# LiyaoTang/contrastBoundary

Hardware: AMD Instinct MI355X
Metric: points/sec through KNN+group+KPConv+CBL block, S3DIS N=40960 K=16 (higher is better)
Workload: dtype f32

## Files before the change

contrastboundary_amd/build.py:

```python
import concurrent.futures
import os
import shutil
import subprocess
import sys

PKG = os.path.dirname(os.path.abspath(__file__))
CSRC = os.path.join(PKG, "csrc")
LIBDIR = os.path.join(PKG, "lib")
OBJDIR = os.path.join(LIBDIR, "obj")
SO = os.path.join(LIBDIR, "libcbl_amd.so")
INCLUDE = os.path.join(os.path.dirname(PKG), "include")

HIPCC = shutil.which("hipcc") or "/opt/rocm/bin/hipcc"
FLAGS = ["--offload-arch=gfx950", "-O3", "-std=c++17", "-fPIC", "-ffp-contract=off", "-munsafe-fp-atomics",
         "-fvisibility=hidden", "-Wall", "-Wno-unused-function", "-I" + INCLUDE, "-I" + CSRC]


def sources():
    return sorted(os.path.join(CSRC, f) for f in os.listdir(CSRC) if f.endswith(".hip"))


def headers():
    hs = [os.path.join(CSRC, f) for f in os.listdir(CSRC) if f.endswith(".h")]
    hs += [os.path.join(INCLUDE, f) for f in os.listdir(INCLUDE) if f.endswith(".h")]
    return hs


EXTRA_FLAGS = {"local_aggregation.hip": ["-mllvm", "-amdgpu-mfma-vgpr-form"]}

def _compile(src, obj, verbose):
    tmp = obj + ".tmp.%d" % os.getpid()
    cmd = [HIPCC] + FLAGS + EXTRA_FLAGS.get(os.path.basename(src), []) + ["-c", src, "-o", tmp]
    if verbose:
        print(" ".join(cmd), flush=True)
    r = subprocess.run(cmd, capture_output=True, text=True)
    if r.returncode != 0:
        raise RuntimeError("hipcc failed for %s:\n%s\n%s" % (src, r.stdout, r.stderr))
    if verbose and r.stderr.strip():
        print(r.stderr)
    os.replace(tmp, obj)


def is_stale():
    if not os.path.exists(SO):
        return True
    t = os.path.getmtime(SO)
    return any(os.path.getmtime(p) > t for p in sources() + headers())


def build(force=False, verbose=False):
    import fcntl
    os.makedirs(OBJDIR, exist_ok=True)
    with open(os.path.join(LIBDIR, ".build.lock"), "w") as lock:
        fcntl.flock(lock, fcntl.LOCK_EX)
        try:
            if not force and not is_stale():
                return SO
            return _build_locked(force, verbose)
        finally:
            fcntl.flock(lock, fcntl.LOCK_UN)


def _build_locked(force, verbose):
    hdr_time = max([os.path.getmtime(h) for h in headers()] + [os.path.getmtime(__file__)])
    jobs, objs = [], []
    for src in sources():
        obj = os.path.join(OBJDIR, os.path.basename(src)[:-4] + ".o")
        objs.append(obj)
        if force or not os.path.exists(obj) or os.path.getmtime(obj) < max(os.path.getmtime(src), hdr_time):
            jobs.append((src, obj))
    if jobs:
        with concurrent.futures.ThreadPoolExecutor(max_workers=min(8, len(jobs))) as ex:
            for f in [ex.submit(_compile, s, o, verbose) for s, o in jobs]:
                f.result()
    if jobs or not os.path.exists(SO):
        tmp = SO + ".tmp.%d" % os.getpid()
        cmd = [HIPCC, "--offload-arch=gfx950", "-shared", "-fPIC", "-o", tmp] + objs
        if verbose:
            print(" ".join(cmd), flush=True)
        r = subprocess.run(cmd, capture_output=True, text=True)
        if r.returncode != 0:
            raise RuntimeError("link failed:\n%s\n%s" % (r.stdout, r.stderr))
        os.replace(tmp, SO)
    else:
        os.utime(SO)
    return SO


if __name__ == "__main__":
    print(build(force="--force" in sys.argv, verbose="--verbose" in sys.argv))
```

contrastboundary_amd/hotpath.py:

```python
import os
import sys

import torch

from . import heads, local_aggregation, pointops

KP = 15
CBL_NSAMPLE = 36
CBL_DIM = 32


class Scene:

    def __init__(self, xyz, feat, labels, offset):
        self.xyz, self.feat, self.labels, self.offset = xyz, feat, labels, offset
        self.n, self.c = feat.shape

    @staticmethod
    def synthetic_numpy(n, c, seed=0, b=1):
        import numpy as np
        from . import synthetic as S
        xyz, labels = S.s_room(n, seed, scale=1.0 if n <= 100000 else float(np.sqrt(n / 40000.0)))
        rng = np.random.default_rng(seed + 1000)
        feat = rng.normal(size=(n, c)).astype(np.float32)
        off = S.offsets(n, b, seed)
        kpts = (rng.normal(size=(KP, 3)) * 0.06).astype(np.float32); kpts[0] = 0
        kw = (rng.normal(size=(KP, c)) / np.sqrt(KP)).astype(np.float32)
        latent = rng.normal(size=(n, CBL_DIM)).astype(np.float32)
        return dict(xyz=xyz, feat=feat, labels=labels, offset=off, kernel_points=kpts, kernel_weights=kw, latent=latent)

    @staticmethod
    def upstream_numpy(n, c, k, seed=0):
        import numpy as np
        rng = np.random.default_rng(seed + 2000)
        return dict(grad_grouped=rng.normal(size=(n, k, 3 + c)).astype(np.float32), grad_kpconv=rng.normal(size=(n, c)).astype(np.float32))

    @staticmethod
    def synthetic(n, c, seed=0, b=1, device="cuda"):
        a = Scene.synthetic_numpy(n, c, seed, b)
        t = lambda v: torch.from_numpy(v).to(device)
        sc = Scene(t(a["xyz"]), t(a["feat"]), t(a["labels"]), t(a["offset"]))
        sc.kernel_points, sc.kernel_weights, sc.latent = t(a["kernel_points"]), t(a["kernel_weights"]), t(a["latent"])
        sc.seed = seed
        return sc

    def upstream(self, k):
        cache = self.__dict__.setdefault("_upstream", {})
        if k not in cache:
            a = Scene.upstream_numpy(self.n, self.c, k, getattr(self, "seed", 0))
            cache[k] = {name: torch.from_numpy(v).to(self.xyz.device) for name, v in a.items()}
        return cache[k]


SIDE_STAGES = ("cbl_knnquery_k%d" % CBL_NSAMPLE,)


def stages(scene, k=16, backward=False, pair_tables=False):
    n, c = scene.n, scene.c
    st = []
    leaf = (lambda t: t.detach().requires_grad_(True)) if backward else (lambda t: t)
    if backward:
        scene.upstream(k)

    def knn(s):
        s["idx"], s["dist2"] = pointops.knnquery_raw(k, scene.xyz, scene.xyz, scene.offset, scene.offset)
    st.append(("knnquery_k%d" % k, knn, 12 * n + 12 * n + 8 * n * k, 8.0 * n * n))

    def group(s):
        s["feat_leaf"], s["kw_leaf"] = leaf(scene.feat), leaf(scene.kernel_weights)
        s["grouped"] = pointops.queryandgroup(k, scene.xyz, scene.xyz, s["feat_leaf"], s["idx"], scene.offset, scene.offset, use_xyz=True)
    st.append(("queryandgroup", group, 4 * n * k + 12 * n + 12 * n + 4 * n * c + 4 * n * k * (3 + c), 3.0 * n * k))

    extent = 0.12

    def kpconv(s):
        s["kpconv"] = local_aggregation.kpconv(scene.xyz, scene.xyz, s["idx"], s["feat_leaf"], scene.kernel_points, s["kw_leaf"], extent)
    st.append(("kpconv_fwd", kpconv, 12 * n + 12 * n + 4 * n * c + 4 * n * k + 4 * n * c, 2.0 * n * k * KP * c + 2.0 * n * KP * c))

    d = CBL_DIM

    def cbl_knn(s):
        s["cbl_idx"], _ = pointops.knnquery_raw(CBL_NSAMPLE, scene.xyz, scene.xyz, scene.offset, scene.offset, algo="set")
    st.append(("cbl_knnquery_k%d" % CBL_NSAMPLE, cbl_knn, 24 * n + 8 * n * CBL_NSAMPLE, 8.0 * n * n))

    def cbl_transpose(s):
        s["cbl_transposed"] = pointops.neighbor_transpose(s["cbl_idx"], n, companion=s.get("idx") if (pair_tables and backward) else None)
    st.append(("cbl_neighbor_transpose", cbl_transpose, 8 * n * CBL_NSAMPLE + 4 * (n + 1), 0.0))

    def cbl_fwd(s):
        s["cbl_latent"] = scene.latent.detach().requires_grad_(True)
        s["cbl_loss"] = heads.point_contrast(s["cbl_latent"], scene.labels, s["cbl_idx"], 1.0, 0.1)
    st.append(("cbl_mining_loss_fwd", cbl_fwd, 4 * n * CBL_NSAMPLE + 4 * n * d + 4 * n + 8 * n + 4 * n * CBL_NSAMPLE + 4 * n * d,
               1.0 * n * (CBL_NSAMPLE - 1) * (8 * d + 50)))

    def cbl_bwd(s):
        s["cbl_grad"], = torch.autograd.grad(s["cbl_loss"], s["cbl_latent"])
    st.append(("cbl_mining_loss_bwd", cbl_bwd, 4 * (n + 1) + 8 * n * CBL_NSAMPLE + 12 * n * d, 3.0 * n * (CBL_NSAMPLE - 1) * d))
    if not backward:
        return st

    def transpose(s):
        s["transposed"] = pointops.neighbor_transpose(s["idx"], n)
    st.append(("neighbor_transpose_k%d" % k, transpose, 8 * n * k + 4 * (n + 1), 0.0))

    def group_bwd(s):
        s["grad_feat_group"], = torch.autograd.grad(s["grouped"], s["feat_leaf"], scene.upstream(k)["grad_grouped"])
    st.append(("queryandgroup_bwd", group_bwd, 4 * n * k + 4 * n * k * c + 4 * n * c, 1.0 * n * k * c))

    def kpconv_bwd(s):
        s["grad_feat_kpconv"], s["grad_kernel_weights"] = torch.autograd.grad(s["kpconv"], (s["feat_leaf"], s["kw_leaf"]), scene.upstream(k)["grad_kpconv"])
    st.append(("kpconv_bwd", kpconv_bwd, 12 * n + 12 * n + 4 * n * c + 4 * n * k + 4 * n * c + 4 * n * c + 4 * KP * c,
               2.0 * (2.0 * n * k * KP * c + 2.0 * n * KP * c)))
    return st


def pt_layer(scene, seed=0):
    from . import blocks
    cache = scene.__dict__.setdefault("_pt_layer", {})
    if seed not in cache:
        torch.manual_seed(1234 + seed)
        cache[seed] = blocks.PointTransformerLayer(scene.c, scene.c, 8, 16).to(scene.xyz.device).train()
    return cache[seed]


def stages_pt(scene, k=16, backward=False, pair_tables=False):
    n, c = scene.n, scene.c
    layer = pt_layer(scene)
    layer.nsample = k
    params = [p for p in layer.parameters()]
    st = []
    if backward:
        scene.upstream(k)

    def knn(s):
        s["idx"], s["dist2"] = pointops.knnquery_raw(k, scene.xyz, scene.xyz, scene.offset, scene.offset)
    st.append(("knnquery_k%d" % k, knn, 12 * n + 12 * n + 8 * n * k, 8.0 * n * n))

    def layer_fwd(s):
        s["feat_leaf"] = scene.feat.detach().requires_grad_(True) if backward else scene.feat
        s["pt_out"] = layer([scene.xyz, s["feat_leaf"], scene.offset], idx=s["idx"])
    st.append(("pt_layer_fwd", layer_fwd, 12 * n + 12 * n * c + 4 * n * k + 4 * n * c,
               2.0 * n * k * (9 + 3 * c + c * c / 8.0 + c * c / 64.0) + 6.0 * n * c * c))

    d = CBL_DIM

    def cbl_knn(s):
        s["cbl_idx"], _ = pointops.knnquery_raw(CBL_NSAMPLE, scene.xyz, scene.xyz, scene.offset, scene.offset, algo="set")
    st.append(("cbl_knnquery_k%d" % CBL_NSAMPLE, cbl_knn, 24 * n + 8 * n * CBL_NSAMPLE, 8.0 * n * n))

    def cbl_transpose(s):
        s["cbl_transposed"] = pointops.neighbor_transpose(s["cbl_idx"], n, companion=s.get("idx") if (pair_tables and backward) else None)
    st.append(("cbl_neighbor_transpose", cbl_transpose, 8 * n * CBL_NSAMPLE + 4 * (n + 1), 0.0))

    def cbl_fwd(s):
        s["cbl_latent"] = scene.latent.detach().requires_grad_(True)
        s["cbl_loss"] = heads.point_contrast(s["cbl_latent"], scene.labels, s["cbl_idx"], 1.0, 0.1)
    st.append(("cbl_mining_loss_fwd", cbl_fwd, 4 * n * CBL_NSAMPLE + 4 * n * d + 4 * n + 8 * n + 4 * n * CBL_NSAMPLE + 4 * n * d,
               1.0 * n * (CBL_NSAMPLE - 1) * (8 * d + 50)))

# ... 315 lines not shown
```

contrastboundary_amd/local_aggregation.py:

```python
import collections
import ctypes

import torch
from torch.autograd import Function

from . import _lib

_i = ctypes.c_int
_f = ctypes.c_float


def _chk(t, dtype, name):
    if not (isinstance(t, torch.Tensor) and t.is_cuda and t.dtype == dtype and t.is_contiguous()):
        raise TypeError(f"{name}: expected a contiguous CUDA tensor of {dtype}")
    return t


class _KPConv(Function):
    @staticmethod
    def forward(ctx, query_points, support_points, neighbors_indices, features, kernel_points, kernel_weights, extent, influence, closest):
        n, K = neighbors_indices.shape
        n0, C = features.shape
        KP = kernel_points.shape[0]
        out = torch.empty((n, C), dtype=torch.float32, device=features.device)
        from . import pointops
        order = pointops.spatial_order(query_points)
        _lib.check(_lib.lib().cbl_kpconv_forward_ordered(_i(n), _i(n0), _i(K), _i(C), _i(KP), _lib.ptr(query_points), _lib.ptr(support_points),
                                                         _lib.ptr(neighbors_indices), _lib.ptr(features), _lib.ptr(kernel_points), _lib.ptr(kernel_weights),
                                                         _f(extent), _i(influence), _i(closest), _lib.ptr(order), _lib.ptr(out),
                                                         _lib.stream_of(features)), "cbl_kpconv_forward")
        ctx.save_for_backward(query_points, support_points, neighbors_indices, features, kernel_points, kernel_weights)
        ctx.cfg = (extent, influence, closest)
        return out

    @staticmethod
    def backward(ctx, grad_out):
        q, s, idx, f, kp, kw = ctx.saved_tensors
        extent, influence, closest = ctx.cfg
        n, K = idx.shape
        n0, C = f.shape
        grad_out = grad_out.contiguous()
        L = _lib.lib()
        from . import pointops
        tr = None
        if C % 4 == 0:
            tr = pointops.neighbor_transpose(idx, n0, build=pointops._build_table(n * K))
        if tr is not None:
            order, inv_start, inv_src = tr
            gf = torch.empty_like(f) if ctx.needs_input_grad[3] else None
            gkw = torch.empty_like(kw) if ctx.needs_input_grad[5] else None
            need = L.cbl_kpconv_backward_csr_workspace_bytes(_i(n0), _i(C), _i(kp.shape[0])) if gkw is not None else 0
            ws = torch.empty(max(need, 1), dtype=torch.uint8, device=f.device)
            rc = L.cbl_kpconv_backward_csr(_i(n), _i(n0), _i(K), _i(C), _i(kp.shape[0]), _lib.ptr(q), _lib.ptr(s), _lib.ptr(f), _lib.ptr(kp), _lib.ptr(kw),
                                           _f(extent), _i(influence), _i(closest), _lib.ptr(grad_out), _lib.ptr(order), _lib.ptr(inv_start), _lib.ptr(inv_src),
                                           _lib.ptr(gf), _lib.ptr(gkw), _lib.ptr(ws), ctypes.c_size_t(ws.numel()), _lib.stream_of(f))
            if rc != _lib.ERR_UNSUPPORTED:
                _lib.check(rc, "cbl_kpconv_backward_csr")
                return None, None, None, gf, None, gkw, None, None, None
        gf = torch.zeros_like(f) if ctx.needs_input_grad[3] else None
        gkw = torch.zeros_like(kw) if ctx.needs_input_grad[5] else None
        _lib.check(L.cbl_kpconv_backward(_i(n), _i(n0), _i(K), _i(C), _i(kp.shape[0]), _lib.ptr(q), _lib.ptr(s), _lib.ptr(idx), _lib.ptr(f),
                                         _lib.ptr(kp), _lib.ptr(kw), _f(extent), _i(influence), _i(closest), _lib.ptr(grad_out),
                                         _lib.ptr(gf), _lib.ptr(gkw), _lib.stream_of(f)), "cbl_kpconv_backward")
        return None, None, None, gf, None, gkw, None, None, None


def kpconv(query_points, support_points, neighbors_indices, features, kernel_points, kernel_weights, extent,
           KP_influence="linear", convolution_mode="sum"):
    _chk(query_points, torch.float32, "query_points"); _chk(support_points, torch.float32, "support_points")
    _chk(neighbors_indices, torch.int32, "neighbors_indices"); _chk(features, torch.float32, "features")
    _chk(kernel_points, torch.float32, "kernel_points"); _chk(kernel_weights, torch.float32, "kernel_weights")
    if KP_influence not in ("linear", "constant"):
        raise NotImplementedError("KP_influence 'gaussian': radius_gaussian is not defined in the reference")
    if convolution_mode not in ("sum", "closest"):
        raise ValueError("Unknown convolution mode. Should be 'closest' or 'sum'")
    return _KPConv.apply(query_points, support_points, neighbors_indices, features, kernel_points, kernel_weights, float(extent),
                         1 if KP_influence == "linear" else 0, 1 if convolution_mode == "closest" else 0)


class _AdaptiveWeight(Function):
    @staticmethod
    def forward(ctx, query_points, support_points, neighbors_indices, features, fc_weight, fc_bias, radius, reduction_mean):
        n, K = neighbors_indices.shape
        n0, C = features.shape
        L = _lib.lib()
        pad = torch.empty(1, dtype=torch.int32, device=features.device)
        if reduction_mean:
            _lib.check(L.cbl_index_max(ctypes.c_longlong(n * K), _lib.ptr(neighbors_indices), _lib.ptr(pad), _lib.stream_of(features)), "cbl_index_max")
        out = torch.empty((n, C), dtype=torch.float32, device=features.device)
        from . import pointops
        order = pointops.spatial_order(query_points)
        _lib.check(L.cbl_adaptive_weight_forward_ordered(_i(n), _i(n0), _i(K), _i(C), _lib.ptr(query_points), _lib.ptr(support_points), _lib.ptr(neighbors_indices),
                                                         _lib.ptr(features), _f(radius), _lib.ptr(fc_weight), _lib.ptr(fc_bias), _lib.ptr(pad), _i(reduction_mean),
                                                         _lib.ptr(order), _lib.ptr(out), _lib.stream_of(features)), "cbl_adaptive_weight_forward")
        ctx.save_for_backward(query_points, support_points, neighbors_indices, features, fc_weight, fc_bias, pad)
        ctx.cfg = (radius, reduction_mean)
        return out

    @staticmethod
    def backward(ctx, grad_out):
        q, s, idx, f, w, b, pad = ctx.saved_tensors
        radius, reduction_mean = ctx.cfg
        n, K = idx.shape
        n0, C = f.shape
        grad_out = grad_out.contiguous()
        L = _lib.lib()
        need_f, need_w, need_b = ctx.needs_input_grad[3], ctx.needs_input_grad[4], ctx.needs_input_grad[5]
        from . import pointops
        tr = None
        if C % 4 == 0:
            tr = pointops.neighbor_transpose(idx, n0, build=pointops._build_table(n * K))
        if tr is not None:
            order, inv_start, inv_src = tr
            gf = torch.empty_like(f) if need_f else None
            gw = torch.empty_like(w) if need_w else None
            gb = torch.empty_like(b) if need_b else None
            ws = torch.empty(L.cbl_adaptive_weight_backward_csr_workspace_bytes(_i(n), _i(n0), _i(C)), dtype=torch.uint8, device=f.device)
            rc = L.cbl_adaptive_weight_backward_csr(_i(n), _i(n0), _i(K), _i(C), _lib.ptr(q), _lib.ptr(s), _lib.ptr(idx), _lib.ptr(f), _f(radius), _lib.ptr(w),
                                                    _lib.ptr(b), _lib.ptr(pad), _i(reduction_mean), _lib.ptr(grad_out), _lib.ptr(order), _lib.ptr(inv_start),
                                                    _lib.ptr(inv_src), _lib.ptr(gf), _lib.ptr(gw), _lib.ptr(gb), _lib.ptr(ws), ctypes.c_size_t(ws.numel()),
                                                    _lib.stream_of(f))
            if rc != _lib.ERR_UNSUPPORTED:
                _lib.check(rc, "cbl_adaptive_weight_backward_csr")
                return None, None, None, gf, gw, gb, None, None
        gf = torch.zeros_like(f) if need_f else None
        gw = torch.zeros_like(w) if need_w else None
        gb = torch.zeros_like(b) if need_b else None
        _lib.check(L.cbl_adaptive_weight_backward(_i(n), _i(n0), _i(K), _i(C), _lib.ptr(q), _lib.ptr(s), _lib.ptr(idx), _lib.ptr(f), _f(radius),
                                                  _lib.ptr(w), _lib.ptr(b), _lib.ptr(pad), _i(reduction_mean), _lib.ptr(grad_out),
                                                  _lib.ptr(gf), _lib.ptr(gw), _lib.ptr(gb), _lib.stream_of(f)), "cbl_adaptive_weight_backward")
        return None, None, None, gf, gw, gb, None, None


def adaptive_weight(query_points, support_points, neighbors_indices, features, radius, fc_weight, fc_bias, reduction="mean"):
    _chk(query_points, torch.float32, "query_points"); _chk(support_points, torch.float32, "support_points")
    _chk(neighbors_indices, torch.int32, "neighbors_indices"); _chk(features, torch.float32, "features")
    _chk(fc_weight, torch.float32, "fc_weight"); _chk(fc_bias, torch.float32, "fc_bias")
    if reduction not in ("mean", "avg", "sum"):
        raise NotImplementedError(f"Reduction {reduction} not supported in the fused AdaptiveWeight")
    return _AdaptiveWeight.apply(query_points, support_points, neighbors_indices, features, fc_weight, fc_bias, float(radius),
                                 1 if reduction in ("mean", "avg") else 0)


POSPOOL_EMBEDDINGS = {"one": 0, "xyz": 1, "distance": 2, "exp_-d": 3, "direction_exp_-d": 4, "direction_d": 5, "sin_cos": 6,
                      "two_order": 7, "three_order": 8}
_POSPOOL_REDUCTIONS = {"sum": 0, "mean": 1, "avg": 1, "max": 2}


class _PosPool(Function):
    @staticmethod
    def forward(ctx, query_points, support_points, neighbors_indices, features, radius, pe, red):
        n, K = neighbors_indices.shape
        n0, C = features.shape
        L = _lib.lib()
        pad = torch.empty(1, dtype=torch.int32, device=features.device)
        if red == 1:
            _lib.check(L.cbl_index_max(ctypes.c_longlong(n * K), _lib.ptr(neighbors_indices), _lib.ptr(pad), _lib.stream_of(features)), "cbl_index_max")
        out = torch.empty((n, C), dtype=torch.float32, device=features.device)
        _lib.check(L.cbl_pospool_forward(_i(n), _i(n0), _i(K), _i(C), _lib.ptr(query_points), _lib.ptr(support_points), _lib.ptr(neighbors_indices),
                                         _lib.ptr(features), _f(radius), _i(pe), _i(red), _lib.ptr(pad), _lib.ptr(out), _lib.stream_of(features)),
# ... 302 lines not shown
```

include/cbl_amd.h:

```cpp
#ifndef CBL_AMD_H
#define CBL_AMD_H

#include <stddef.h>
#include <stdint.h>

#ifdef __cplusplus
extern "C" {
#endif

#define CBL_OK               0
#define CBL_ERR_BAD_ARG     (-1)
#define CBL_ERR_WORKSPACE   (-2)
#define CBL_ERR_UNSUPPORTED (-3)

#define CBL_KNN_MAX_NSAMPLE 1024
#define CBL_CONTRAST_PAIRS_MAX_D 4096

const char* cbl_version(void);
int         cbl_device_arch_ok(void);


int cbl_knnquery(int b, int n, int m, int nsample,
                 const float* xyz, const float* new_xyz,
                 const int* offset, const int* new_offset,
// ... 74 lines not shown
int cbl_aggregation_forward(int n, int nsample, int c, int w_c, const float* input, const float* position, const float* weight, const int* idx, float* output, void* stream);
int cbl_aggregation_forward_ordered(int n, int nsample, int c, int w_c, const float* input, const float* position, const float* weight, const int* idx,
                                    const int* order, float* output, void* stream);
int cbl_aggregation_backward(int n, int nsample, int c, int w_c, const float* input, const float* position, const float* weight, const int* idx, const float* grad_output, float* grad_input, float* grad_position, float* grad_weight, void* stream);


int cbl_queryandgroup(int m, int nsample, int c, int use_xyz, const float* xyz, const float* new_xyz, const float* feat, const int* idx, float* out, void* stream);
int cbl_queryandgroup_ordered(int m, int nsample, int c, int use_xyz, const float* xyz, const float* new_xyz, const float* feat, const int* idx,
                              const int* order, float* out, void* stream);

int cbl_interpolation_weights(int n, int k, const float* dist2, float* weight, float* dist, void* stream);



int cbl_subscene_label(int m, int kr, int num_classes, const long long* target, const int* neighbor_idx, float* out, void* stream);

int cbl_label_argmax(int m, int num_classes, const float* labels, int* amax, void* stream);

int cbl_point_contrast_forward(int m, int nsample, int d, const float* features, const int* amax, const int* neighbor_idx,
                               float temperature, float weight, float* per_point, int* point_mask, float* stats, float* loss, void* stream);
int cbl_point_contrast_backward(int m, int nsample, int d, const float* features, const int* amax, const int* neighbor_idx,
                                float temperature, float weight, const float* stats, const float* grad_loss, float* grad_features, void* stream);

int cbl_point_contrast_forward_grad(int m, int nsample, int d, const float* features, const int* amax, const int* neighbor_idx,
                                    float temperature, float weight, float* per_point, int* point_mask, float* stats, float* loss,
                                    float* grad_unit, void* stream);
int cbl_point_contrast_forward_l64(int m, int nsample, int d, const float* features, const long long* labels, const int* neighbor_idx,
                                   float temperature, float weight, float* per_point, int* point_mask, float* stats, float* loss, void* stream);
int cbl_point_contrast_forward_grad_l64(int m, int nsample, int d, const float* features, const long long* labels, const int* neighbor_idx,
                                        float temperature, float weight, float* per_point, int* point_mask, float* stats, float* loss,
                                        float* grad_unit, void* stream);
int cbl_tf_contrast_forward_grad(int m, int n_valid, int nsample, int d, const float* features, const int* labels, const int* neighbors,
                                 float temperature, float weight, float* per_point, int* point_mask, float* stats, float* loss,
                                 float* grad_unit, void* stream);
int cbl_tf_contrast_forward_kl(int m, int n_valid, int nsample, int d, const float* features, const float* soft_labels, int num_classes,
                               float kl_threshold, const int* neighbors, float temperature, float weight, float* per_point, int* point_mask,
                               float* stats, float* loss, void* stream);
int cbl_tf_contrast_forward_grad_kl(int m, int n_valid, int nsample, int d, const float* features, const float* soft_labels, int num_classes,
                                    float kl_threshold, const int* neighbors, float temperature, float weight, float* per_point, int* point_mask,
                                    float* stats, float* loss, float* grad_unit, void* stream);
int cbl_contrast_grad_scale(long long total, const float* grad_unit, const float* stats, const float* grad_loss, float weight,
                            float* grad_features, void* stream);

int cbl_contrast_pairs_forward(int m, int n_valid, int flags, int nsample, int d, const float* features, const void* labels, int num_classes,
                               float kl_threshold, const int* neighbor_idx, const int* order, float temperature, float weight,
                               float* per_point, int* point_mask, float* stats, float* loss, float* coef, float* grad_own, void* stream);
#define CBL_ROLE_LABEL 0
#define CBL_ROLE_POS 1
#define CBL_ROLE_NEG 2
#define CBL_ROLE_NEG_REJECT 3
int cbl_contrast_pairs_forward_samples(int m, int n_valid, int flags, int nsample, int d, const float* features, const void* labels, int num_classes,
                                       float kl_threshold, const int* sample_idx, const unsigned char* roles, const unsigned char* sample_valid,
                                       const int* order, float temperature, float weight, float* per_point, int* point_mask, float* stats,
                                       float* loss, float* coef, float* grad_own, void* stream);
int cbl_contrast_pairs_backward(int m, int nsample, int d, const float* features, const float* coef, const float* grad_own, const int* order,
                                const int* inv_start, const int* inv_src, const float* stats, const float* grad_loss, float weight,
                                float* grad_features, void* stream);

int cbl_contrast_pairs_backward_atomic(int m, int n_valid, int nsample, int d, const float* features, const float* coef, const float* grad_own,
                                       const int* neighbor_idx, const float* stats, const float* grad_loss, float weight,
                                       float* grad_features, void* stream);

int cbl_tf_contrast_forward(int m, int n_valid, int nsample, int d, const float* features, const int* labels, const int* neighbors,
                            float temperature, float weight, float* per_point, int* point_mask, float* stats, float* loss, void* stream);
int cbl_tf_contrast_backward(int m, int n_valid, int nsample, int d, const float* features, const int* labels, const int* neighbors,
                             float temperature, float weight, const float* stats, const float* grad_loss, float* grad_features, void* stream);
int cbl_tf_scene_label(int m, int n_valid, int k, int num_classes, const long long* point_labels, const int* scene_neighbor, int by_valid, float* out, void* stream);

int cbl_boundary_mask(int n, int k, const long long* labels, const int* neighbor_idx, unsigned char* bound, unsigned char* plain, int* cnt, void* stream);

int cbl_cumulate_probs(int n, int num_classes, int m, const long long* inds, const float* pred, float smooth, int mode, float* probs,
                       int* scratch_n, void* stream);

int cbl_boundary_iou(int n, int k, int num_classes, long long ignore_label, const long long* pred, const long long* labels,
                     const int* neighbor_idx, unsigned long long* hist, void* stream);


int cbl_kpconv_forward(int n, int n0, int K, int C, int KP, const float* query_points, const float* support_points, const int* neighbors_indices,
                       const float* features, const float* kernel_points, const float* kernel_weights, float extent, int influence, int closest,
                       float* out, void* stream);
int cbl_kpconv_forward_ordered(int n, int n0, int K, int C, int KP, const float* query_points, const float* support_points, const int* neighbors_indices,
                               const float* features, const float* kernel_points, const float* kernel_weights, float extent, int influence, int closest,
                               const int* order, float* out, void* stream);
int cbl_kpconv_backward(int n, int n0, int K, int C, int KP, const float* query_points, const float* support_points, const int* neighbors_indices,
                        const float* features, const float* kernel_points, const float* kernel_weights, float extent, int influence, int closest,
                        const float* grad_out, float* grad_features, float* grad_kernel_weights, void* stream);

size_t cbl_kpconv_backward_csr_workspace_bytes(int n0, int C, int KP);
int cbl_kpconv_backward_csr(int n, int n0, int K, int C, int KP, const float* query_points, const float* support_points, const float* features,
                            const float* kernel_points, const float* kernel_weights, float extent, int influence, int closest,
                            const float* grad_out, const int* order_dst, const int* inv_start, const int* inv_src,
                            float* grad_features, float* grad_kernel_weights, void* workspace, size_t workspace_bytes, void* stream);

int cbl_index_max(long long total, const int* idx, int* out_max, void* stream);
int cbl_adaptive_weight_forward(int n, int n0, int K, int C, const float* query_points, const float* support_points, const int* neighbors_indices,
                                const float* features, float radius, const float* fc_weight, const float* fc_bias, const int* padding_num,
                                int reduction_mean, float* out, void* stream);
int cbl_adaptive_weight_forward_ordered(int n, int n0, int K, int C, const float* query_points, const float* support_points, const int* neighbors_indices,
                                        const float* features, float radius, const float* fc_weight, const float* fc_bias, const int* padding_num,
                                        int reduction_mean, const int* order, float* out, void* stream);
int cbl_adaptive_weight_backward(int n, int n0, int K, int C, const float* query_points, const float* support_points, const int* neighbors_indices,
                                 const float* features, float radius, const float* fc_weight, const float* fc_bias, const int* padding_num,
                                 int reduction_mean, const float* grad_out, float* grad_features, float* grad_fc_weight, float* grad_fc_bias, void* stream);

size_t cbl_adaptive_weight_backward_csr_workspace_bytes(int n, int n0, int C);
int cbl_adaptive_weight_backward_csr(int n, int n0, int K, int C, const float* query_points, const float* support_points, const int* neighbors_indices,
                                     const float* features, float radius, const float* fc_weight, const float* fc_bias, const int* padding_num,
                                     int reduction_mean, const float* grad_out, const int* order_dst, const int* inv_start, const int* inv_src,
                                     float* grad_features, float* grad_fc_weight, float* grad_fc_bias, void* workspace, size_t workspace_bytes, void* stream);

int cbl_pospool_forward(int n, int n0, int K, int C, const float* query_points, const float* support_points, const int* neighbors_indices,
                        const float* features, float radius, int position_embedding, int reduction, const int* padding_num,
                        float* out, void* stream);
int cbl_pospool_backward(int n, int n0, int K, int C, const float* query_points, const float* support_points, const int* neighbors_indices,
                         const float* features, float radius, int position_embedding, int reduction, const int* padding_num,
                         const float* grad_out, float* grad_features, void* stream);
size_t cbl_pospool_backward_csr_workspace_bytes(int n);
int cbl_pospool_backward_csr(int n, int n0, int K, int C, const float* query_points, const float* support_points, const int* neighbors_indices,
                             float radius, int position_embedding, int reduction, const int* padding_num, const float* grad_out,
                             const int* order_dst, const int* inv_start, const int* inv_src, float* grad_features,
                             void* workspace, size_t workspace_bytes, void* stream);

size_t cbl_pointwise_mlp_workspace_bytes(int n, int n0, int K, int C_out);
int cbl_pointwise_mlp_forward(int n, int n0, int K, int C_out, const float* query_points, const float* support_points, const int* neighbors_indices,
                              const float* center_term, const float* neighbor_term, const float* w_pos, float radius,
                              int bn_mode, const float* gamma, const float* beta, float eps, float momentum, float* moving_mean, float* moving_var,
                              int activation, int reduction, const int* padding_num, float* save_mean, float* save_invstd, float* out,
                              void* workspace, size_t workspace_bytes, void* stream);
int cbl_pointwise_mlp_backward_csr(int n, int n0, int K, int C_out, const float* query_points, const float* support_points, const int* neighbors_indices,
                                   const float* center_term, const float* neighbor_term, const float* w_pos, float radius,
                                   int bn_mode, const float* gamma, const float* beta, const float* save_mean, const float* save_invstd,
                                   int activation, int reduction, const int* padding_num, const float* out, const float* grad_out,
                                   const int* order_dst, const int* inv_start, const int* inv_src,
                                   float* grad_center, float* grad_neighbor, float* grad_w_pos, float* grad_gamma, float* grad_beta,
                                   void* workspace, size_t workspace_bytes, void* stream);

size_t cbl_attn_workspace_bytes(int C, int G);
int cbl_attn_w2_forward(int n, int K, int C, int G, const float* x_q, const float* x_k, const int* idx, const float* p1,
                        const float* W3C, const float* b3C, const float* bn_weight, const float* bn_bias, float eps, float momentum,
                        float* running_mean, float* running_var, long long* num_batches_tracked, int training,
                        const float* Wa, const float* ba, float* save_mean, float* save_invstd, float* w2,
                        void* workspace, size_t workspace_bytes, void* stream);
int cbl_attn_w2_backward(int n, int K, int C, int G, const float* x_q, const float* x_k, const int* idx, const float* p1,
                         const float* W3C, const float* b3C, const float* bn_weight, const float* bn_bias,
                         const float* save_mean, const float* save_invstd, const float* Wa, const float* grad_w2,
                         float* grad_xq, float* grad_xk, float* grad_p1, float* grad_W3C, float* grad_b3C,
                         float* grad_bn_weight, float* grad_bn_bias, float* grad_Wa, float* grad_ba,
                         void* workspace, size_t workspace_bytes, void* stream);
int cbl_attn_agg_forward(int n, int K, int C, int G, const float* x_v, const int* idx, const float* p1, const float* W3C, const float* b3C,
                         const float* a, float* out, void* stream);
int cbl_attn_agg_backward(int n, int K, int C, int G, const float* x_v, const int* idx, const float* p1, const float* W3C, const float* b3C,
                          const float* a, const float* grad_out, float* grad_xv, float* grad_p1, float* grad_W3C, float* grad_b3C, float* grad_a,
                          void* workspace, size_t workspace_bytes, void* stream);
int cbl_attn_agg_softmax_forward(int n, int K, int C, int G, const float* x_v, const int* idx, const float* p1, const float* W3C, const float* b3C,
                                 const float* logits, float* a, float* out, void* stream);
int cbl_attn_agg_softmax_backward(int n, int K, int C, int G, const float* x_v, const int* idx, const float* p1, const float* W3C, const float* b3C,
                                  const float* a, const float* grad_out, float* grad_xv, float* grad_p1, float* grad_W3C, float* grad_b3C,
                                  float* grad_logits, void* workspace, size_t workspace_bytes, void* stream);

int cbl_attn_w2_backward_csr(int n, int K, int C, int G, const float* x_q, const float* x_k, const int* idx, const float* p1,
                             const float* W3C, const float* b3C, const float* bn_weight, const float* bn_bias,
                             const float* save_mean, const float* save_invstd, const float* Wa, const float* grad_w2,
                             const int* order, const int* inv_start, const int* inv_src,
                             float* grad_xq, float* grad_xk, float* grad_p1, float* grad_W3C, float* grad_b3C,
                             float* grad_bn_weight, float* grad_bn_bias, float* grad_Wa, float* grad_ba,
                             void* workspace, size_t workspace_bytes, void* stream);
// ... 161 lines not shown
```

Before: 147.1 million.

## Fuse query-and-group gather with KPConv forward into one MFMA kernel

Adds a fused HIP kernel that gathers neighbour features and relative coordinates once per point, writes the grouped tensor, and computes the KPConv forward from the same registers and LDS using 16x16x4 f32 MFMA. The stage pipeline now runs this fused path in the group stage and reuses its KPConv output in the kpconv stage, so neighbour features are not gathered a second time. Autograd wrappers reuse the existing backward routines. It is limited to C=64, K=16, KP<=16 and sum mode, and it adds a spatial_order call plus more register pressure in exchange.

```diff
diff --git a/contrastboundary_amd/build.py b/contrastboundary_amd/build.py
--- a/contrastboundary_amd/build.py
+++ b/contrastboundary_amd/build.py
@@ -26,7 +26,7 @@
     return hs
 
 
-EXTRA_FLAGS = {"local_aggregation.hip": ["-mllvm", "-amdgpu-mfma-vgpr-form"]}
+EXTRA_FLAGS = {"local_aggregation.hip": ["-mllvm", "-amdgpu-mfma-vgpr-form"], "group_kpconv.hip": ["-mllvm", "-amdgpu-mfma-vgpr-form"]}
 
 def _compile(src, obj, verbose):
     tmp = obj + ".tmp.%d" % os.getpid()
diff --git a/contrastboundary_amd/csrc/group_kpconv.hip b/contrastboundary_amd/csrc/group_kpconv.hip
--- /dev/null
+++ b/contrastboundary_amd/csrc/group_kpconv.hip
@@ -0,0 +1,32 @@
+#include "cbl_common.h"
+
+namespace {
+#include "group_kpconv_pipe.h"
+
+#ifndef GKP_AHEAD
+#define GKP_AHEAD 0
+#endif
+}
+
+CBL_EXPORT int cbl_queryandgroup_kpconv_forward_ordered(int m, int n0, int nsample, int c, int use_xyz, int KP, const float* xyz, const float* new_xyz,
+                                                        const float* feat, const int* idx, const float* kernel_points, const float* kernel_weights,
+                                                        float extent, int influence, int closest, const int* order, float* grouped, float* out, void* stream)
+{
+    if (m < 0 || n0 < 0 || nsample <= 0 || c <= 0 || KP <= 0 || !(extent > 0.f) || influence < 0 || influence > 1) return CBL_ERR_BAD_ARG;
+    if (m == 0) return CBL_OK;
+    if (!xyz || !new_xyz || !feat || !idx || !kernel_points || !kernel_weights || !grouped || !out) return CBL_ERR_BAD_ARG;
+    const bool aligned = cbl_host_aligned16(feat) && cbl_host_aligned16(grouped) && cbl_host_aligned16(out) && cbl_host_aligned16(kernel_weights);
+    const bool fits = (long long)m * nsample < 0xffffffffLL && (unsigned long long)n0 * c * 4ull < (1ull << 32);
+    if (!(use_xyz && c == 64 && nsample == 16 && KP <= 16 && !closest && aligned && fits)) return CBL_ERR_UNSUPPORTED;
+    const unsigned npieces = (unsigned)m, nwg = (npieces + 3) / 4;
+    auto grid_of = [&](const void* fn) -> unsigned {
+        const unsigned g = cbl_resident_blocks(fn, 256, 0);
+        return g < cbl_round_up8(nwg) ? g : cbl_round_up8(nwg);
+    };
+#define CBL_GKP(LI) hipLaunchKernelGGL((group_kpconv_fwd_kernel<LI, GKP_AHEAD != 0>), dim3(grid_of(reinterpret_cast<const void*>(&group_kpconv_fwd_kernel<LI, GKP_AHEAD != 0>))), \
+                                       dim3(256), 0, cbl_stream(stream), npieces, KP, xyz, new_xyz, reinterpret_cast<const float4*>(feat), idx, order, kernel_points,         \
+                                       kernel_weights, extent, grouped, out)
+    if (influence) CBL_GKP(true); else CBL_GKP(false);
+#undef CBL_GKP
+    return cbl_status();
+}
diff --git a/contrastboundary_amd/csrc/group_kpconv_pipe.h b/contrastboundary_amd/csrc/group_kpconv_pipe.h
--- /dev/null
+++ b/contrastboundary_amd/csrc/group_kpconv_pipe.h
@@ -0,0 +1,134 @@
+#pragma once
+#include <gather_wave.h>
+#include <group_kpconv_wave.h>
+
+constexpr int GKP_WAVES = 4;
+
+template <bool LINEAR, bool AHEAD>
+__global__ __launch_bounds__(256) void group_kpconv_fwd_kernel(unsigned npieces, int KP, const float* __restrict__ xyz, const float* __restrict__ new_xyz,
+                                                               const float4* __restrict__ feat, const int* __restrict__ idx, const int* __restrict__ order,
+                                                               const float* __restrict__ kpts, const float* __restrict__ kw, float extent,
+                                                               float* __restrict__ grouped, float* __restrict__ out)
+{
+    constexpr int C4T = 16, PR = 16, C = 4 * C4T;
+    constexpr int oc = C + 3, NL = PR * C4T / 64, NCH = PR * oc / 4, NS = (NCH + 63) / 64;
+    static_assert((PR * oc) % 4 == 0 && 3 * PR <= 64, "pieces are whole 16-byte chunks, one wave load holds a piece's coordinates");
+    __shared__ __attribute__((aligned(16))) float gk_lds[GKP_WAVES * PR * oc];
+    __shared__ float4 gk_kw[16 * 16];
+    {
+        const int row = threadIdx.x >> 4, col = threadIdx.x & 15;
+        gk_kw[threadIdx.x] = row < KP ? *reinterpret_cast<const float4*>(kw + (size_t)row * C + 4 * col) : make_float4(0.f, 0.f, 0.f, 0.f);
+    }
+    __syncthreads();
+    const int lane = threadIdx.x & 63, wv = gw_uniform((int)(threadIdx.x >> 6));
+    const int kp_id = lane & 15, kq = lane >> 4;
+    const bool kp_ok = kp_id < KP;
+    const float kx = kp_ok ? kpts[3 * kp_id] : 0.f, ky = kp_ok ? kpts[3 * kp_id + 1] : 0.f, kz = kp_ok ? kpts[3 * kp_id + 2] : 0.f;
+    const float inv_extent = 1.0f / extent;
+    const float m2kx = -2.f * kx, m2ky = -2.f * ky, m2kz = -2.f * kz, k2 = (kx * kx + ky * ky) + kz * kz;
+    float* piece = gk_lds + wv * PR * oc;
+    const unsigned nwg = (npieces + 3) >> 2, vend = 8 * cbl_xcd_per(nwg), vstep = gridDim.x;
+    auto piece_of = [&](unsigned v) -> int {
+        const unsigned t = (v < vend ? cbl_xcd_slot(v, nwg) : 0u) * 4 + wv;
+        const bool ok = v < vend && t < npieces;
+        const int pt = order ? order[ok ? t : 0u] : (int)t;
+        return gw_uniform(ok ? pt : -1);
+    };
+    auto ids_of = [&](int pc) -> int { return idx[(size_t)(pc < 0 ? 0 : pc) * PR + (lane < PR ? lane : 0)]; };
+    float4 v[NL]; float cs, cq;
+    auto load_piece = [&](float4 (&r)[NL], int ids, int pc) {
+        const int pq = pc < 0 ? 0 : pc;
+#pragma unroll
+        for (int j = 0; j < NL; j++) {
+            const int f = lane + 64 * j, row = f / C4T, part = f % C4T;
+            r[j] = feat[(size_t)gw_shfl(ids, row) * C4T + part];
+        }
+        const int ec = lane < 3 * PR ? lane : 0, row = ec / 3, a = ec - 3 * row;
+        cs = xyz[(size_t)gw_shfl(ids, row) * 3 + a];
+        cq = new_xyz[(size_t)pq * 3 + a];
+    };
+    auto park = [&]() {
+#pragma unroll
+        for (int j = 0; j < NL; j++) {
+            const int f = lane + 64 * j, row = f / C4T, part = f % C4T;
+            float* d = piece + row * oc + 3 + 4 * part;
+            d[0] = v[j].x; d[1] = v[j].y; d[2] = v[j].z; d[3] = v[j].w;
+        }
+        const int row = lane / 3, a = lane - 3 * row;
+        if (lane < 3 * PR) piece[row * oc + a] = cs - cq;
+    };
+    auto kpconv = [&](int pc) {
+        gw_wave_sync();
+        const float* rel = piece + kp_id * oc;
+        const float mrx = rel[0], mry = rel[1], mrz = rel[2];
+        const float mr2 = (mrx * mrx + mry * mry) + mrz * mrz;
+        float a[NL];
+#pragma unroll
+        for (int gi = 0; gi < NL; gi++) {
+            const int src = 4 * gi + kq;
+            const float rx = gk_shfl(mrx, src), ry = gk_shfl(mry, src), rz = gk_shfl(mrz, src), r2 = gk_shfl(mr2, src);
+            const float sq = fmaxf(__builtin_fmaf(m2kx, rx, __builtin_fmaf(m2ky, ry, __builtin_fmaf(m2kz, rz, r2 + k2))), 0.f);
+            const float w = LINEAR ? fmaxf(1.0f - gk_sqrt(sq) * inv_extent, 0.0f) : 1.0f;
+            a[gi] = kp_ok ? w : 0.f;
+        }
+        const gk_f32x4 zero = {0.f, 0.f, 0.f, 0.f};
+        gk_f32x4 acc[4];
+#pragma unroll
+        for (int t = 0; t < 4; t++) acc[t] = zero;
+#pragma unroll
+        for (int gi = 0; gi < NL; gi++) {
+            acc[0] = gk_mfma(a[gi], v[gi].x, acc[0]);
+            acc[1] = gk_mfma(a[gi], v[gi].y, acc[1]);
+            acc[2] = gk_mfma(a[gi], v[gi].z, acc[2]);
+            acc[3] = gk_mfma(a[gi], v[gi].w, acc[3]);
+        }
+        float res[4];
+#pragma unroll
+        for (int t = 0; t < 4; t++) res[t] = 0.f;
+#pragma unroll
+        for (int r = 0; r < 4; r++) {
+            const float4 k4 = gk_kw[(kq * 4 + r) * 16 + kp_id];
+            res[0] = __builtin_fmaf(k4.x, acc[0][r], res[0]); res[1] = __builtin_fmaf(k4.y, acc[1][r], res[1]);
+            res[2] = __builtin_fmaf(k4.z, acc[2][r], res[2]); res[3] = __builtin_fmaf(k4.w, acc[3][r], res[3]);
+        }
+#pragma unroll
+        for (int t = 0; t < 4; t++) res[t] = gk_rows_sum4(res[t]);
+        if (lane < 16) *reinterpret_cast<float4*>(out + (size_t)pc * C + 4 * kp_id) = make_float4(res[0], res[1], res[2], res[3]);
+    };
+    int p0 = piece_of(blockIdx.x), p1 = piece_of(blockIdx.x + vstep), p2 = piece_of(blockIdx.x + 2 * vstep);
+    int id1 = ids_of(p1);
+    load_piece(v, ids_of(p0), p0);
+    int pc = -1;
+    auto turn = [&](unsigned vnext) {
+        park();
+        pc = p0;
+        p0 = p1; const int idn = id1; p1 = p2;
+        id1 = ids_of(p1);
+        p2 = piece_of(vnext);
+        if (AHEAD) {
+            float4 vn[NL];
+            load_piece(vn, idn, p0);
+            __builtin_amdgcn_sched_barrier(0);
+            if (pc >= 0) kpconv(pc);
+#pragma unroll
+            for (int j = 0; j < NL; j++) v[j] = vn[j];
+        } else {
+            if (pc >= 0) kpconv(pc);
+            load_piece(v, idn, p0);
+        }
+    };
+    turn(blockIdx.x + 3 * vstep);
+    for (unsigned vv = blockIdx.x; vv < vend; vv += vstep) {
+        gw_wave_sync();
+        {
+            float* o = grouped + (size_t)(pc < 0 ? 0 : pc) * PR * oc;
+#pragma unroll
+            for (int u = 0; u < NS; u++) {
+                const int ch = lane + 64 * u;
+                if (ch < NCH) gw_store16_streaming(o + 4 * ch, piece + 4 * ch);
+            }
+        }
+        gw_wave_sync();
+        turn(vv + 4 * vstep);
+    }
+}
diff --git a/contrastboundary_amd/csrc/group_kpconv_wave.h b/contrastboundary_amd/csrc/group_kpconv_wave.h
--- /dev/null
+++ b/contrastboundary_amd/csrc/group_kpconv_wave.h
@@ -0,0 +1,17 @@
+#pragma once
+#include <hip/hip_runtime.h>
+
+typedef float gk_f32x4 __attribute__((ext_vector_type(4)));
+
+__device__ __forceinline__ float gk_shfl(float v, int src_lane) { return __shfl(v, src_lane); }
+__device__ __forceinline__ float gk_sqrt(float x) { return __builtin_amdgcn_sqrtf(x); }
+__device__ __forceinline__ gk_f32x4 gk_mfma(float a, float b, gk_f32x4 c) { return __builtin_amdgcn_mfma_f32_16x16x4f32(a, b, c, 0, 0, 0); }
+__device__ __forceinline__ float gk_rows_sum4(float x)
+{
+    const unsigned u = __float_as_uint(x);
+    const auto a = __builtin_amdgcn_permlane16_swap(u, u, false, false);
+    const float y = __uint_as_float(a[0]) + __uint_as_float(a[1]);
+    const unsigned w = __float_as_uint(y);
+    const auto b = __builtin_amdgcn_permlane32_swap(w, w, false, false);
+    return __uint_as_float(b[0]) + __uint_as_float(b[1]);
+}
diff --git a/contrastboundary_amd/hotpath.py b/contrastboundary_amd/hotpath.py
--- a/contrastboundary_amd/hotpath.py
+++ b/contrastboundary_amd/hotpath.py
@@ -53,9 +53,10 @@
 
 
 SIDE_STAGES = ("cbl_knnquery_k%d" % CBL_NSAMPLE,)
-
-
-def stages(scene, k=16, backward=False, pair_tables=False):
+_FUSED_KPCONV = "_kpconv_of_fused_forward"
+
+
+def stages(scene, k=16, backward=False, pair_tables=False, fused_forward=True):
     n, c = scene.n, scene.c
     st = []
     leaf = (lambda t: t.detach().requires_grad_(True)) if backward else (lambda t: t)
@@ -66,15 +67,20 @@
         s["idx"], s["dist2"] = pointops.knnquery_raw(k, scene.xyz, scene.xyz, scene.offset, scene.offset)
     st.append(("knnquery_k%d" % k, knn, 12 * n + 12 * n + 8 * n * k, 8.0 * n * n))
 
+    extent = 0.12
+
     def group(s):
         s["feat_leaf"], s["kw_leaf"] = leaf(scene.feat), leaf(scene.kernel_weights)
-        s["grouped"] = pointops.queryandgroup(k, scene.xyz, scene.xyz, s["feat_leaf"], s["idx"], scene.offset, scene.offset, use_xyz=True)
+        s.pop(_FUSED_KPCONV, None)
+        if fused_forward and local_aggregation.group_kpconv_eligible(s["idx"], s["feat_leaf"], scene.kernel_points):
+            s["grouped"], s[_FUSED_KPCONV] = local_aggregation.group_kpconv(scene.xyz, scene.xyz, s["idx"], s["feat_leaf"], scene.kernel_points, s["kw_leaf"], extent)
+        else:
+            s["grouped"] = pointops.queryandgroup(k, scene.xyz, scene.xyz, s["feat_leaf"], s["idx"], scene.offset, scene.offset, use_xyz=True)
     st.append(("queryandgroup", group, 4 * n * k + 12 * n + 12 * n + 4 * n * c + 4 * n * k * (3 + c), 3.0 * n * k))
 
-    extent = 0.12
-
     def kpconv(s):
-        s["kpconv"] = local_aggregation.kpconv(scene.xyz, scene.xyz, s["idx"], s["feat_leaf"], scene.kernel_points, s["kw_leaf"], extent)
+        fused = s.pop(_FUSED_KPCONV, None)
+        s["kpconv"] = fused if fused is not None else local_aggregation.kpconv(scene.xyz, scene.xyz, s["idx"], s["feat_leaf"], scene.kernel_points, s["kw_leaf"], extent)
     st.append(("kpconv_fwd", kpconv, 12 * n + 12 * n + 4 * n * c + 4 * n * k + 4 * n * c, 2.0 * n * k * KP * c + 2.0 * n * KP * c))
 
     d = CBL_DIM
diff --git a/contrastboundary_amd/local_aggregation.py b/contrastboundary_amd/local_aggregation.py
--- a/contrastboundary_amd/local_aggregation.py
+++ b/contrastboundary_amd/local_aggregation.py
@@ -76,6 +76,67 @@
         raise ValueError("Unknown convolution mode. Should be 'closest' or 'sum'")
     return _KPConv.apply(query_points, support_points, neighbors_indices, features, kernel_points, kernel_weights, float(extent),
                          1 if KP_influence == "linear" else 0, 1 if convolution_mode == "closest" else 0)
+
+
+class _GroupedOfFusedForward(Function):
+
+    @staticmethod
+    def forward(ctx, xyz, new_xyz, feat, idx, use_xyz, grouped):
+        ctx.save_for_backward(idx)
+        ctx.dims = (xyz.shape[0], feat.shape[0], feat.shape[1], use_xyz)
+        return grouped
+
+    @staticmethod
+    def backward(ctx, grad_out):
+        from . import pointops
+        return pointops._QueryAndGroup.backward(ctx, grad_out) + (None,)
+
+
+class _KPConvOfFusedForward(Function):
+
+    @staticmethod
+    def forward(ctx, query_points, support_points, neighbors_indices, features, kernel_points, kernel_weights, extent, influence, closest, out):
+        ctx.save_for_backward(query_points, support_points, neighbors_indices, features, kernel_points, kernel_weights)
+        ctx.cfg = (extent, influence, closest)
+        return out
+
+    @staticmethod
+    def backward(ctx, grad_out):
+        return _KPConv.backward(ctx, grad_out) + (None,)
+
+
+def group_kpconv_eligible(neighbors_indices, features, kernel_points, convolution_mode="sum"):
+    return (features.dim() == 2 and features.shape[1] == 64 and neighbors_indices.dim() == 2 and neighbors_indices.shape[1] == 16
+            and kernel_points.shape[0] <= 16 and convolution_mode == "sum")
+
+
+def group_kpconv(query_points, support_points, neighbors_indices, features, kernel_points, kernel_weights, extent,
+                 KP_influence="linear", convolution_mode="sum"):
+    from . import pointops
+    q, s, idx, f = query_points, support_points, neighbors_indices, features
+    _chk(q, torch.float32, "query_points"); _chk(s, torch.float32, "support_points")
+    _chk(idx, torch.int32, "neighbors_indices"); _chk(f, torch.float32, "features")
+    _chk(kernel_points, torch.float32, "kernel_points"); _chk(kernel_weights, torch.float32, "kernel_weights")
+    if KP_influence not in ("linear", "constant"):
+        raise NotImplementedError("KP_influence 'gaussian': radius_gaussian is not defined in the reference")
+    if convolution_mode not in ("sum", "closest"):
+        raise ValueError("Unknown convolution mode. Should be 'closest' or 'sum'")
+    influence, closest = 1 if KP_influence == "linear" else 0, 1 if convolution_mode == "closest" else 0
+    if group_kpconv_eligible(idx, f, kernel_points, convolution_mode):
+        order = pointops.spatial_order(q)
+        n, K = idx.shape
+        n0, C = f.shape
+        grouped = torch.empty((n, K, 3 + C), dtype=torch.float32, device=f.device)
+        out = torch.empty((n, C), dtype=torch.float32, device=f.device)
+        rc = _lib.lib().cbl_queryandgroup_kpconv_forward_ordered(_i(n), _i(n0), _i(K), _i(C), _i(1), _i(kernel_points.shape[0]), _lib.ptr(s), _lib.ptr(q),
+                                                                 _lib.ptr(f), _lib.ptr(idx), _lib.ptr(kernel_points), _lib.ptr(kernel_weights), _f(float(extent)),
+                                                                 _i(influence), _i(closest), _lib.ptr(order), _lib.ptr(grouped), _lib.ptr(out), _lib.stream_of(f))
+        if rc != _lib.ERR_UNSUPPORTED:
+            _lib.check(rc, "cbl_queryandgroup_kpconv_forward_ordered")
+            return (_GroupedOfFusedForward.apply(s, q, f, idx, True, grouped),
+                    _KPConvOfFusedForward.apply(q, s, idx, f, kernel_points, kernel_weights, float(extent), influence, closest, out))
+    return (pointops.queryandgroup(idx.shape[1], s, q, f, idx, None, None, use_xyz=True),
+            kpconv(q, s, idx, f, kernel_points, kernel_weights, extent, KP_influence, convolution_mode))
 
 
 class _AdaptiveWeight(Function):
diff --git a/include/cbl_amd.h b/include/cbl_amd.h
--- a/include/cbl_amd.h
+++ b/include/cbl_amd.h
@@ -180,6 +180,9 @@
 int cbl_kpconv_forward_ordered(int n, int n0, int K, int C, int KP, const float* query_points, const float* support_points, const int* neighbors_indices,
                                const float* features, const float* kernel_points, const float* kernel_weights, float extent, int influence, int closest,
                                const int* order, float* out, void* stream);
+int cbl_queryandgroup_kpconv_forward_ordered(int m, int n0, int nsample, int c, int use_xyz, int KP, const float* xyz, const float* new_xyz,
+                                             const float* feat, const int* idx, const float* kernel_points, const float* kernel_weights,
+                                             float extent, int influence, int closest, const int* order, float* grouped, float* out, void* stream);
 int cbl_kpconv_backward(int n, int n0, int K, int C, int KP, const float* query_points, const float* support_points, const int* neighbors_indices,
                         const float* features, const float* kernel_points, const float* kernel_weights, float extent, int influence, int closest,
                         const float* grad_out, float* grad_features, float* grad_kernel_weights, void* stream);
```

Result: faster. 154.1 million (median of 6 runs) (+4.7%).
